# gssales/gaussian-splatting-reflection

Hardware: AMD Instinct MI355X
Metric: train_step_views_per_s (fwd+bwd, 1e6 Gaussians @1080p, surfel rasterizer + reflection path) (higher is better)
Workload: dtype f32

## Files before the change

gaussian-splatting-reflection_amd/csrc/gsr_common.hip:

```cpp
#include "gsr_internal.hpp"
#include <cstdarg>
#include <string>
#include <initializer_list>
#include <vector>
#include <mutex>
#include "gsr_sort.hpp"
#include <rocprim/device/device_scan.hpp>
#include <rocprim/iterator/counting_iterator.hpp>
#include <rocprim/iterator/transform_iterator.hpp>

namespace gsr {

static thread_local char g_err[512] = "";
void set_error(const char* fmt, ...) {
	va_list ap;
	va_start(ap, fmt);
	vsnprintf(g_err, sizeof(g_err), fmt, ap);
	va_end(ap);
}


struct ProfRec {
	int stage;
	hipEvent_t e0, e1;
};
static bool g_prof_on = false;
static std::vector<ProfRec*> g_prof_recs;
static std::vector<ProfRec*> g_prof_free;
static std::mutex g_prof_mu;

StageTimer::StageTimer(int stage_, hipStream_t stream_) : stage(stage_), stream(stream_), rec(nullptr) {
	if (!g_prof_on) return;
	std::lock_guard<std::mutex> lk(g_prof_mu);
	ProfRec* r = nullptr;
	if (!g_prof_free.empty()) {
		r = g_prof_free.back();
		g_prof_free.pop_back();
	} else {
		r = new ProfRec();
		if (hipEventCreate(&r->e0) != hipSuccess || hipEventCreate(&r->e1) != hipSuccess) { delete r; return; }
	}
	r->stage = stage;
	(void)hipEventRecord(r->e0, stream);
	rec = r;
}
StageTimer::~StageTimer() {
	if (!rec) return;
	ProfRec* r = (ProfRec*)rec;
	(void)hipEventRecord(r->e1, stream);
	std::lock_guard<std::mutex> lk(g_prof_mu);
	g_prof_recs.push_back(r);
}

static int g_opt_cull = 1;
int option_cull() { return g_opt_cull; }
static int g_opt_dev = 0;
int option_dev() { return g_opt_dev; }
unsigned long long* dev_pair_counter() {
	static std::mutex mu;
	static unsigned long long* words[64];
	int dev = 0;
	if (hipGetDevice(&dev) != hipSuccess || dev < 0 || dev >= 64) return nullptr;
	std::lock_guard<std::mutex> lk(mu);
	if (!words[dev]) {
		if (hipMalloc((void**)&words[dev], sizeof(unsigned long long)) != hipSuccess) { (void)hipGetLastError(); words[dev] = nullptr; return nullptr; }
		if (hipMemset(words[dev], 0, sizeof(unsigned long long)) != hipSuccess) return nullptr;
	}
	return words[dev];
}
static int g_opt_emit_items = 0;
static int g_opt_mailbox = 1;
static int option_mailbox() { return g_opt_mailbox; }
static int g_opt_sort_driver = GSR_ONESWEEP_DRIVER;
int option_sort_driver() { return GSR_ONESWEEP_DRIVER && g_opt_sort_driver; }

uint32_t higher_msb(uint32_t n) {
	uint32_t msb = sizeof(n) * 4;
	uint32_t step = msb;
	while (step > 1) {
		step /= 2;
		if (n >> msb) msb += step;
		else msb -= step;
	}
	if (n >> msb) msb++;
	return msb;
}

using SortConfig = rocprim::radix_sort_config<rocprim::default_config, rocprim::default_config, rocprim::default_config, 65536>;
#ifndef DEPTH_SORT_BS
#define DEPTH_SORT_BS 1024
#endif
#ifndef DEPTH_SORT_IPT
#define DEPTH_SORT_IPT 4
#endif
#define DEPTH_SORT_SHAPE DEPTH_SORT_BS, DEPTH_SORT_IPT, 8
#define DEPTH_KEY_BITS 31u
#define DEPTH_KEY_PLACES 4u
#ifndef TILE_SORT_IPT
#define TILE_SORT_IPT 16
#endif
#ifndef TILE_SORT_BITS
#define TILE_SORT_BITS 8
#endif
#ifndef TILE_SORT_BS
#define TILE_SORT_BS 1024
#endif
#define TILE_SORT_SHAPE TILE_SORT_BS, TILE_SORT_IPT, TILE_SORT_BITS
#ifndef TILE_SORT_SMALL_FROM
#define TILE_SORT_SMALL_FROM 9000000
#endif
#define TILE_SORT_SHAPE_SMALL TILE_SORT_BS, (TILE_SORT_IPT / 2), TILE_SORT_BITS
#define TILE_SORT_SHAPE_SMALL7 TILE_SORT_BS, (TILE_SORT_IPT / 2), 7
static bool tile_sort_small(size_t R) { return R >= (size_t)TILE_SORT_SMALL_FROM; }
static bool tile_sort_7bit(size_t R, int end_bit) { return tile_sort_small(R) && end_bit > 7 && end_bit <= 14; }
template <class F>
static auto with_tile_sort(size_t R, int end_bit, F&& f) {
	if (tile_sort_7bit(R, end_bit)) return f(RadixSort<TILE_SORT_SHAPE_SMALL7, SortConfig>{});
	if (tile_sort_small(R)) return f(RadixSort<TILE_SORT_SHAPE_SMALL, SortConfig>{});
	return f(RadixSort<TILE_SORT_SHAPE, SortConfig>{});
}
using DepthSort = RadixSort<DEPTH_SORT_SHAPE, SortConfig>;
// ... 518 lines not shown

extern "C" int gsr_set_option(const char* name, int value) {
	if (!name) { set_error("gsr_set_option: NULL option name"); return GSR_E_INVALID; }
	if (std::string(name) == "cull") { g_opt_cull = value ? 1 : 0; return 0; }
	if (std::string(name) == "dev") { g_opt_dev = value; return 0; }
	if (std::string(name) == "emit_items") { g_opt_emit_items = (value == 1 || value == 2) ? value : 0; return 0; }
	if (std::string(name) == "mailbox") { g_opt_mailbox = value ? 1 : 0; return 0; }
	if (std::string(name) == "sort_driver") { g_opt_sort_driver = value ? 1 : 0; return 0; }
	set_error("gsr_set_option: unknown option '%s'", name);
	return GSR_E_INVALID;
}
extern "C" int gsr_profile_enable(int on) {
	std::lock_guard<std::mutex> lk(g_prof_mu);
	for (ProfRec* r : g_prof_recs) g_prof_free.push_back(r);
	g_prof_recs.clear();
	g_prof_on = on != 0;
	return 0;
}
extern "C" int gsr_profile_collect(float* ms_out, int* launches_out) {
	std::lock_guard<std::mutex> lk(g_prof_mu);
	for (int i = 0; i < GSR_STAGE_COUNT; i++) { if (ms_out) ms_out[i] = 0.f; if (launches_out) launches_out[i] = 0; }
	for (ProfRec* r : g_prof_recs) {
		float ms = 0.f;
		if (hipEventSynchronize(r->e1) == hipSuccess && hipEventElapsedTime(&ms, r->e0, r->e1) == hipSuccess) {
			if (ms_out) ms_out[r->stage] += ms;
			if (launches_out) launches_out[r->stage] += 1;
		}
		g_prof_free.push_back(r);
	}
	g_prof_recs.clear();
	return 0;
}

extern "C" int gsr_mark_visible(int P, const float* means3D, const float* viewmatrix, const float* projmatrix, uint8_t* present,
                                void* stream_) {
	(void)projmatrix;
	hipStream_t stream = (hipStream_t)stream_;
	if (P < 0 || (P > 0 && (!means3D || !viewmatrix || !present))) { set_error("gsr_mark_visible: invalid argument"); return GSR_E_INVALID; }
	if (P == 0) return 0;
	mark_visible_kernel<<<(P + 255) / 256, 256, 0, stream>>>(P, means3D, viewmatrix, present);
	GSR_LAUNCH_CHECK(0, stream);
	return 0;
}

extern "C" int gsr_debug_fetch(int variant, const char* name, int P, int R, int width, int height, const void* geom_buffer,
                               const void* binning_buffer, const void* image_buffer, void* dst, void* stream_) {
	hipStream_t stream = (hipStream_t)stream_;
	if ((variant != 0 && variant != 1) || !name || P < 0 || R < 0 || width <= 0 || height <= 0) {
		set_error("gsr_debug_fetch: invalid argument (variant 0 or 1, a name, P >= 0, R >= 0, width, height)");
		return GSR_E_INVALID;
	}
	{
		static const struct { const char* name; int buf; } arrays[] = {
			{"pairs", -1}, {"depths", 0}, {"means2D", 0}, {"tiles_touched", 0}, {"cull", 0}, {"point_offsets", 0}, {"clamped", 0}, {"rgb", 0}, {"geom4", 0},
			{"transMat", 0}, {"cov3D", 0}, {"point_list", 1}, {"blend_mask", 1}, {"keys", 1}, {"ranges", 2}, {"final_T", 2}, {"n_contrib", 2}};
		int buf = -2;
		for (const auto& a : arrays) if (strcmp(a.name, name) == 0) buf = a.buf;
		if (buf == -2 || (strcmp(name, "transMat") == 0 && variant != 0)) { set_error("gsr_debug_fetch: unknown array '%s'", name); return GSR_E_INVALID; }
		const bool reads = buf == -1 || (buf == 0 && P > 0) || (buf == 1 && (R > 0 || strcmp(name, "blend_mask") == 0)) || buf == 2;
		const void* src = buf == 0 ? geom_buffer : buf == 1 ? binning_buffer : buf == 2 ? image_buffer : dst;
		if (reads && (!dst || !src || (strcmp(name, "keys") == 0 && !geom_buffer))) { set_error("gsr_debug_fetch: '%s' needs its workspace buffer and dst", name); return GSR_E_INVALID; }
	}
	const int tiles_x = (width + 15) / 16, tiles_y = (height + 15) / 16;
	const size_t HW = (size_t)width * height, tiles = (size_t)tiles_x * tiles_y;
	const WorkspaceLayout& layout = variant == 0 ? SURFEL_LAYOUT : GAUSS_LAYOUT;
	const int stride = layout.rec_f4 * 4;
	GeomState g = carve_geom((void*)geom_buffer, P, layout, nullptr);
	ImageState im = carve_image((void*)image_buffer, HW, tiles, layout, nullptr);
	BinningState b = carve_binning((void*)binning_buffer, R, tiles, 0, nullptr);
	auto d2d = [&](const void* src, size_t bytes) -> int {
		if (bytes == 0) return 0;
		GSR_HIP_CHECK(hipMemcpyAsync(dst, src, bytes, hipMemcpyDeviceToDevice, stream));
		return 0;
	};
	auto gather = [&](int first, int nf) -> int {
		if (P == 0) return 0;
		gather_rec_kernel<<<(P * nf + 255) / 256, 256, 0, stream>>>(P, (const float*)g.rec, stride, first, nf, (float*)dst);
		GSR_LAUNCH_CHECK(0, stream);
		return 0;
	};
	std::string n(name);
	if (n == "pairs") {
		const unsigned long long* word = dev_pair_counter();
		if (!word) { set_error("gsr_debug_fetch: no pair counter"); return GSR_E_HIP; }
		return d2d(word, sizeof(unsigned long long));
	}
	if (n == "depths") return d2d(g.depths, (size_t)P * 4);
	if (n == "means2D") return gather(0, 2);

	if (n == "tiles_touched") return d2d(g.tiles_touched, (size_t)P * 4);
	if (n == "cull") return d2d(g.bbox, (size_t)P * 32);
	if (n == "point_offsets") {
		if (P == 0) return 0;
		size_t tmp = (size_t)(static_cast<char*>(g.depth_sort_temp) - static_cast<char*>(g.scan_temp));
		GSR_HIP_CHECK(rocprim::inclusive_scan(g.scan_temp, tmp, g.tiles_touched, g.point_offsets, (size_t)P, rocprim::plus<uint32_t>(), stream, false));
		return d2d(g.point_offsets, (size_t)P * 4);
	}
	if (n == "clamped") {
		if (P == 0) return 0;
		widen_clamped_kernel<<<(P + 255) / 256, 256, 0, stream>>>(P, g.clamped, (uint8_t*)dst);
		GSR_LAUNCH_CHECK(0, stream);
		return 0;
	}
	auto pick = [&](std::initializer_list<int> pos) -> int {
		if (P == 0) return 0;
		RecPick pk;
		pk.n = (int)pos.size();
		int i = 0;
		for (int v : pos) pk.pos[i++] = v;
		pick_rec_kernel<<<(P * pk.n + 255) / 256, 256, 0, stream>>>(P, (const float*)g.rec, stride, pk, (float*)dst);
		GSR_LAUNCH_CHECK(0, stream);
		return 0;
	};
	if (n == "rgb") return variant == 0 ? gather(16, 3) : gather(6, 3);
	if (n == "geom4") {
		return variant == 0 ? pick({12, 13, 14, 11}) : gather(2, 4);
	}
	if (n == "transMat" && variant == 0) return pick({2, 4, 6, 3, 5, 7, 8, 9, 10});
	if (n == "cov3D" && variant == 1) { set_error("gsr_debug_fetch: the 3D covariance is not kept by the forward (round 4: the backward recomputes it)"); return GSR_E_INVALID; }
	if (n == "point_list") return d2d(b.point_list, (size_t)R * 4);
	if (n == "blend_mask") return d2d(b.blend_mask, 16 * b.mask_stride * sizeof(unsigned long long));
	if (n == "keys") {
		if (R == 0) return 0;
		rebuild_keys_kernel<<<(R + 255) / 256, 256, 0, stream>>>(R, b.tile_keys, b.point_list, g.depths, (uint64_t*)dst);
		GSR_LAUNCH_CHECK(0, stream);
		return 0;
	}
	if (n == "ranges") return d2d(im.ranges, tiles * 8);
	if (n == "final_T") return d2d(im.final_T, HW * 4 * layout.planes_T);
	if (n == "n_contrib") return d2d(im.n_contrib, HW * 4 * layout.planes_n);
	set_error("gsr_debug_fetch: unknown array '%s'", name);
	return GSR_E_INVALID;
}
```

gaussian-splatting-reflection_amd/csrc/gsr_internal.hpp:

```cpp
#pragma once
#include <cstring>
#include <cstdint>
#include <cstdio>
#include <hip/hip_runtime.h>
#include "../../include/gsr_hip.h"

#define GSR_TILE 16
#define GSR_TILE_PIX 256

namespace gsr {

void set_error(const char* fmt, ...);
#define GSR_HIP_CHECK(expr)                                                                       \
	do {                                                                                          \
		hipError_t _e = (expr);                                                                   \
		if (_e != hipSuccess) {                                                                   \
			gsr::set_error("%s failed: %s (%s:%d)", #expr, hipGetErrorString(_e), __FILE__, __LINE__); \
			return GSR_E_HIP;                                                                     \
		}                                                                                         \
	} while (0)
#define GSR_LAUNCH_CHECK(debug, stream)                                  \
	do {                                                                 \
		GSR_HIP_CHECK(hipGetLastError());                                \
		if (debug) GSR_HIP_CHECK(hipStreamSynchronize(stream));          \
// ... 83 lines not shown
ImageState carve_image(void* buf, size_t HW, size_t tiles, const WorkspaceLayout& layout, size_t* total);
BinningState carve_binning(void* buf, size_t R, size_t tiles, size_t sort_temp_bytes, size_t* total, bool blend_masks = true);
int forward_workspace(gsr_alloc_fn alloc, void* alloc_user, const WorkspaceLayout& layout, size_t P, size_t HW, size_t tiles, GeomState* geom,
                      ImageState* img);

static inline int check_sh_input(const char* entry, int D, int M, const float* shs) {
	if (D < 0 || D > 3 || (shs && (D + 1) * (D + 1) > M)) { set_error("%s: SH degree %d not supported with M=%d", entry, D, M); return GSR_E_INVALID; }
	if (shs && ((M * 3) & 3) == 0 && misaligned16(shs)) {
		set_error("%s: shs (rows of a multiple of 16 bytes) must be 16-byte aligned (float4 accesses); got %p", entry, (const void*)shs);
		return GSR_E_INVALID;
	}
	return 0;
}

struct RasterCam {
	const float* view;
	const float* proj;
	const float* campos;
	int W, H;
	float tan_fovx, tan_fovy, focal_x, focal_y;
};
static inline RasterCam make_cam(const float* view, const float* proj, const float* campos, int W, int H, float tan_fovx, float tan_fovy) {
	RasterCam c;
	c.view = view; c.proj = proj; c.campos = campos; c.W = W; c.H = H;
	c.tan_fovx = tan_fovx; c.tan_fovy = tan_fovy;
	c.focal_y = H / (2.0f * tan_fovy);
	c.focal_x = W / (2.0f * tan_fovx);
	return c;
}

struct BackwardWorkspace { GeomState geom; ImageState img; BinningState bin; int tiles_x, ntiles; };
static inline int backward_prologue(const char* entry, const char* func, const WorkspaceLayout& layout, int P, int M, int R, int width, int height,
                                    bool missing_pointer, const float* shs, const float* dL_dsh, const float* dL_drot, const float* also_aligned,
                                    const char* also_what, void* geom_buffer, void* binning_buffer, void* image_buffer, hipStream_t stream,
                                    BackwardWorkspace* w) {
	if (P < 0 || R < 0 || width <= 0 || height <= 0) { set_error("%s: invalid size", entry); return GSR_E_INVALID; }
	if (P == 0) return 0;
	if (missing_pointer) { set_error("%s: missing required pointer", entry); return GSR_E_INVALID; }
	if (shs && ((M * 3) & 3) == 0) GSR_REQUIRE_ALIGNED16_IN(func, dL_dsh, "dL_dsh");
	GSR_REQUIRE_ALIGNED16_IN(func, dL_drot, "dL_drot");
	GSR_REQUIRE_ALIGNED16_IN(func, also_aligned, also_what);
	w->tiles_x = (width + 15) / 16;
	w->ntiles = w->tiles_x * ((height + 15) / 16);
	w->geom = carve_geom(geom_buffer, P, layout, nullptr);
	w->img = carve_image(image_buffer, (size_t)width * height, w->ntiles, layout, nullptr);
	w->bin = carve_binning(binning_buffer, R, w->ntiles, 0, nullptr);
	GSR_HIP_CHECK(hipMemsetAsync(w->geom.acc, 0, (size_t)P * layout.acc_floats * sizeof(float), stream));
	return 1;
}

int option_cull();
int option_dev();
unsigned long long* dev_pair_counter();
size_t sort_temp_bytes(size_t R, int end_bit);
int run_tile_order(const ImageState& img, size_t tiles, hipStream_t stream);
uint32_t higher_msb(uint32_t n);

int run_binning(gsr_alloc_fn alloc, void* alloc_user, int P, int tiles_x, int tiles_y, const GeomState& geom,
                const ImageState& img, BinningState* out_binning, int prefiltered, int debug, hipStream_t stream, bool blend_masks = true);

int side_gate_wait(hipStream_t stream);
int refl_scratch_check(const char* entry, uint32_t L, int width, int height, const float* scratch, size_t scratch_floats);
int refl_sort_keys_early(uint32_t L, int width, int height, float* scratch, size_t scratch_floats, const uint32_t* sort_keys, int async, bool gated,
                         hipStream_t stream);

}

#ifdef __HIPCC__
namespace gsr {

__device__ __forceinline__ int f2i(float v) { return (int)v; }

__device__ __forceinline__ void get_rect(float px, float py, int max_radius, int gx, int gy, uint32_t& x0, uint32_t& y0,
                                         uint32_t& x1, uint32_t& y1) {
	const float r = (float)max_radius;
	x0 = (uint32_t)min(gx, max(0, f2i((px - r) / 16.0f)));
	y0 = (uint32_t)min(gy, max(0, f2i((py - r) / 16.0f)));
	x1 = (uint32_t)min(gx, max(0, f2i((px + r + 15.0f) / 16.0f)));
	y1 = (uint32_t)min(gy, max(0, f2i((py + r + 15.0f) / 16.0f)));
}

#define GSR_Q1(CTRL, i) "v_add_f32_dpp %" #i ", %" #i ", %" #i " " CTRL " row_mask:0xf bank_mask:0xf\n\t"
#define GSR_DPPB(CTRL, BANK, dst, src) "v_add_f32_dpp %" #dst ", %" #src ", %" #src " " CTRL " row_mask:0xf bank_mask:" BANK "\n\t"
#define GSR_L1(CTRL, d, a, b) GSR_DPPB(CTRL, "0x3", d, a) GSR_DPPB(CTRL, "0xc", d, b)
__device__ __forceinline__ void row_reduce20(const float* v, float* z) {
	float p0, q0, p1, q1, p2, q2, p3, q3, p4, q4;
	asm volatile("s_nop 1\n\t" GSR_L1("row_mirror", 0, 6, 7) GSR_L1("row_mirror", 1, 8, 9) GSR_L1("row_mirror", 2, 10, 11)
	             GSR_L1("row_mirror", 3, 12, 13) GSR_L1("row_mirror", 4, 14, 15) GSR_L1("row_mirror", 5, 16, 17)
	             : "=&v"(p0), "=&v"(q0), "=&v"(p1), "=&v"(q1), "=&v"(p2), "=&v"(q2)
	             : "v"(v[0]), "v"(v[1]), "v"(v[2]), "v"(v[3]), "v"(v[4]), "v"(v[5]), "v"(v[6]), "v"(v[7]), "v"(v[8]), "v"(v[9]), "v"(v[10]), "v"(v[11]));
	asm volatile("s_nop 1\n\t" GSR_L1("row_mirror", 0, 4, 5) GSR_L1("row_mirror", 1, 6, 7) GSR_L1("row_mirror", 2, 8, 9) GSR_L1("row_mirror", 3, 10, 11)
	             : "=&v"(p3), "=&v"(q3), "=&v"(p4), "=&v"(q4)
	             : "v"(v[12]), "v"(v[13]), "v"(v[14]), "v"(v[15]), "v"(v[16]), "v"(v[17]), "v"(v[18]), "v"(v[19]));
#define GSR_L2(d, a, b) GSR_DPPB("row_half_mirror", "0x5", d, a) GSR_DPPB("row_half_mirror", "0xa", d, b)
#define GSR_QA(CTRL) GSR_Q1(CTRL, 0) GSR_Q1(CTRL, 1) GSR_Q1(CTRL, 2) GSR_Q1(CTRL, 3) GSR_Q1(CTRL, 4)
	asm volatile("s_nop 1\n\t" GSR_L2(0, 5, 6) GSR_L2(1, 7, 8) GSR_L2(2, 9, 10) GSR_L2(3, 11, 12) GSR_L2(4, 13, 14)
	             GSR_QA("quad_perm:[2,3,0,1]") GSR_QA("quad_perm:[1,0,3,2]")
	             : "=&v"(z[0]), "=&v"(z[1]), "=&v"(z[2]), "=&v"(z[3]), "=&v"(z[4])
	             : "v"(p0), "v"(q0), "v"(p1), "v"(q1), "v"(p2), "v"(q2), "v"(p3), "v"(q3), "v"(p4), "v"(q4));
}
__device__ __forceinline__ void row_reduce16(const float* v, float* z) {
	float p0, q0, p1, q1, p2, q2, p3, q3;
	asm volatile("s_nop 1\n\t" GSR_L1("row_mirror", 0, 8, 9) GSR_L1("row_mirror", 1, 10, 11) GSR_L1("row_mirror", 2, 12, 13) GSR_L1("row_mirror", 3, 14, 15)
	             GSR_L1("row_mirror", 4, 16, 17) GSR_L1("row_mirror", 5, 18, 19) GSR_L1("row_mirror", 6, 20, 21) GSR_L1("row_mirror", 7, 22, 23)
	             : "=&v"(p0), "=&v"(q0), "=&v"(p1), "=&v"(q1), "=&v"(p2), "=&v"(q2), "=&v"(p3), "=&v"(q3)
	             : "v"(v[0]), "v"(v[1]), "v"(v[2]), "v"(v[3]), "v"(v[4]), "v"(v[5]), "v"(v[6]), "v"(v[7]), "v"(v[8]), "v"(v[9]), "v"(v[10]), "v"(v[11]),
// ... 17 lines not shown
	for (int k = 0; k < N; k++) lds[k * 65 + lane] = v[k];
	wave_lds_sync();
#pragma unroll
	for (int j = 0; j < N; j++) {
		const int e = lane + 64 * j, r = e / N, k = e - r * N;
		if (r < nrows) {
			const float x = lds[k * 65 + r];
			if (ACC) {
				if (x != 0.f) out[e] += x;
			} else {
				out[e] = x;
			}
		}
	}
	wave_lds_sync();
}
template <int N, bool ACC>
__device__ __forceinline__ void wave_store_rows4(float4* lds, const float4* v, float4* __restrict__ out, int pitch, int col0, int nrows, int lane) {
#pragma unroll
	for (int k = 0; k < N; k++) lds[k * 65 + lane] = v[k];
	wave_lds_sync();
#pragma unroll
	for (int j = 0; j < N; j++) {
		const int e = lane + 64 * j, r = e / N, k = e - r * N;
		if (r < nrows) {
			const float4 x = lds[k * 65 + r];
			float4* o = out + (size_t)r * pitch + col0 + k;
			if (ACC) {
				if (x.x != 0.f || x.y != 0.f || x.z != 0.f || x.w != 0.f) {
					const float4 y = *o;
					*o = make_float4(y.x + x.x, y.y + x.y, y.z + x.z, y.w + x.w);
				}
			} else {
				*o = x;
			}
		}
	}
	wave_lds_sync();
}
template <bool ACC> __device__ __forceinline__ void put(float* p, float v) {
	if (ACC) { if (v != 0.f) *p += v; }
	else *p = v;
}
template <bool ACC> __device__ __forceinline__ void put4(float4* p, float a, float b, float c, float d) {
	if (ACC) {
		if (a != 0.f || b != 0.f || c != 0.f || d != 0.f) {
			const float4 r = *p;
			*p = make_float4(r.x + a, r.y + b, r.z + c, r.w + d);
		}
	} else {
		*p = make_float4(a, b, c, d);
	}
}
__device__ __forceinline__ uint32_t ffbl_raw(uint32_t x) {
	uint32_t r;
	asm("v_ffbl_b32 %0, %1" : "=v"(r) : "v"(x));
	return r;
}
__device__ __forceinline__ int row_reduce_slot(int lane) {
	const int q = (lane >> 2) & 3;
	return ((q & 1) << 1) | (q >> 1);
}

typedef unsigned long long lmask;
#define LMASK(cond) __builtin_amdgcn_ballot_w64(cond)
__device__ __forceinline__ float selm(lmask m, float a, float b) {
	float r;
	asm("v_cndmask_b32 %0, %1, %2, %3" : "=v"(r) : "v"(b), "v"(a), "s"(m));
	return r;
}
__device__ __forceinline__ float selm0(lmask m, float a) {
	float r;
	asm("v_cndmask_b32 %0, 0, %1, %2" : "=v"(r) : "v"(a), "s"(m));
	return r;
}
__device__ __forceinline__ uint32_t selmu(lmask m, uint32_t a, uint32_t b) {
	uint32_t r;
	asm("v_cndmask_b32 %0, %1, %2, %3" : "=v"(r) : "v"(b), "v"(a), "s"(m));
	return r;
}

__device__ __forceinline__ float min_raw(float a, float b) {
	float r;
	asm("v_min_f32 %0, %1, %2" : "=v"(r) : "v"(a), "v"(b));
	return r;
}

__device__ __forceinline__ float row_max4(float a, float b, float c, float d) {
	float p, q, z;
	asm volatile("s_nop 1\n\t"
	             "v_max_f32_dpp %0, %2, %2 row_mirror row_mask:0xf bank_mask:0x3\n\t"
	             "v_max_f32_dpp %0, %3, %3 row_mirror row_mask:0xf bank_mask:0xc\n\t"
	             "v_max_f32_dpp %1, %4, %4 row_mirror row_mask:0xf bank_mask:0x3\n\t"
	             "v_max_f32_dpp %1, %5, %5 row_mirror row_mask:0xf bank_mask:0xc\n\t"
	             : "=&v"(p), "=&v"(q) : "v"(a), "v"(b), "v"(c), "v"(d));
	asm volatile("s_nop 1\n\t"
	             "v_max_f32_dpp %0, %1, %1 row_half_mirror row_mask:0xf bank_mask:0x5\n\t"
	             "v_max_f32_dpp %0, %2, %2 row_half_mirror row_mask:0xf bank_mask:0xa\n\t"
	             "s_nop 1\n\t"
	             "v_max_f32_dpp %0, %0, %0 quad_perm:[2,3,0,1] row_mask:0xf bank_mask:0xf\n\t"
	             "s_nop 1\n\t"
	             "v_max_f32_dpp %0, %0, %0 quad_perm:[1,0,3,2] row_mask:0xf bank_mask:0xf\n\t"
	             : "=&v"(z) : "v"(p), "v"(q));
	return z;
}

// ... 63 lines not shown
```

gaussian-splatting-reflection_amd/csrc/gsr_surfel.hip:

```cpp
#include <type_traits>
#include "gsr_internal.hpp"
#include "gsr_tile_walk.hpp"
#include "gsr_sort.hpp"
#include "gsr_math.hpp"
#include "gsr_refl.hpp"

namespace gsr {

#define SA_COLOR 0
#define SA_REFL 3
#define SA_NORMAL 4
#define SA_OPAC 7
#define SA_T 8
#define SA_MEAN2D 17

#define S_NEAR 0.2f
#define S_FAR 100.0f
#define S_FILTER_INV_SQ 2.0f

__device__ __forceinline__ M3 quat_to_rotmat(const float* __restrict__ q, float& w, float& x, float& y, float& z) {
#pragma clang fp contract(off)
	const float s = 1.0f / sqrtf(q[3] * q[3] + q[0] * q[0] + q[1] * q[1] + q[2] * q[2]);
	w = q[0] * s; x = q[1] * s; y = q[2] * s; z = q[3] * s;
	return m3_make(1.f - 2.f * (y * y + z * z), 2.f * (x * y + w * z), 2.f * (x * z - w * y), 2.f * (x * y - w * z),
// ... 24 lines not shown
	float qw, qx, qy, qz;
	const M3 R = quat_to_rotmat(rot, qw, qx, qy, qz);
	const float s0 = mod * scale[0], s1 = mod * scale[1];
	const float L0[3] = {R.m[0][0] * s0, R.m[0][1] * s0, R.m[0][2] * s0};
	const float L1[3] = {R.m[1][0] * s1, R.m[1][1] * s1, R.m[1][2] * s1};
	const float* pm = cam.proj;
	float AB[4][3];
#pragma unroll
	for (int j = 0; j < 4; j++) {
		AB[j][0] = L0[0] * pm[j] + L0[1] * pm[j + 4] + L0[2] * pm[j + 8];
		AB[j][1] = L1[0] * pm[j] + L1[1] * pm[j + 4] + L1[2] * pm[j + 8];
		AB[j][2] = px * pm[j] + py * pm[j + 4] + pz * pm[j + 8] + pm[j + 12];
	}
	const float Wh = (float)(float(cam.W) / 2.0), Wm = (float)(float(cam.W - 1) / 2.0);
	const float Hh = (float)(float(cam.H) / 2.0), Hm = (float)(float(cam.H - 1) / 2.0);
#pragma unroll
	for (int i = 0; i < 3; i++) {
		T.m[0][i] = AB[0][i] * Wh + AB[3][i] * Wm;
		T.m[1][i] = AB[1][i] * Hh + AB[3][i] * Hm;
		T.m[2][i] = AB[3][i];
	}
	const float* vm = cam.view;
	const float nx = R.m[2][0], ny = R.m[2][1], nz = R.m[2][2];
	normal = f3(vm[0] * nx + vm[4] * ny + vm[8] * nz, vm[1] * nx + vm[5] * ny + vm[9] * nz, vm[2] * nx + vm[6] * ny + vm[10] * nz);
}

__device__ __forceinline__ void surfel_cull_record(const M3& T, float cx, float cy, float opa, float4& c0, float4& c1) {
	c0 = make_float4(cx, cy, 0.f, 0.f);
	c1 = make_float4(0.f, cx, cy, -2.0f);
	if (!(opa >= 1.0f / 255.0f)) return;
	const float c2f = 2.0f * logf(255.0f * opa) * 1.05f + 0.1f;
	c1.w = 0.5f * c2f * 1.02f;
	const double ic2 = 1.0 / (double)c2f;
	const double a00 = T.m[0][0], a01 = T.m[0][1], a02 = T.m[0][2];
	const double a10 = T.m[1][0], a11 = T.m[1][1], a12 = T.m[1][2];
	const double a20 = T.m[2][0], a21 = T.m[2][1], a22 = T.m[2][2];
	const double sigma = a20 * a20 + a21 * a21 - a22 * a22 * ic2;
	if (!(sigma < -1e-6 * a22 * a22 * ic2)) return;
	const double sx = a00 * a20 + a01 * a21 - a02 * a22 * ic2, sy = a10 * a20 + a11 * a21 - a12 * a22 * ic2;
	const double Sxx = a00 * a00 + a01 * a01 - a02 * a02 * ic2, Sxy = a00 * a10 + a01 * a11 - a02 * a12 * ic2,
	             Syy = a10 * a10 + a11 * a11 - a12 * a12 * ic2;
	const double is = 1.0 / sigma;
	const double ex = sx * is, ey = sy * is;
	const double g = -is * 1.0404;
	const double Vxx = (Sxx - sx * sx * is) * g + 0.25, Vxy = (Sxy - sx * sy * is) * g, Vyy = (Syy - sy * sy * is) * g + 0.25;
	const double det = Vxx * Vyy - Vxy * Vxy;
	if (!(Vxx > 0.25) || !(Vyy > 0.25) || !(det > 0.0)) return;
	const float fa = (float)(Vyy / det), fb = (float)(-Vxy / det), fc = (float)(Vxx / det);
	if (!(fa > 0.f) || !(fc > 0.f) || !(fa * fc - fb * fb > 0.f) || !(fabsf((float)ex) < 1e7f) || !(fabsf((float)ey) < 1e7f)) return;
	c0 = make_float4((float)ex, (float)ey, fa, fb);
	c1.x = fc;
}

template <bool TRAIN>
__device__ __forceinline__ bool
surfel_preprocess_one(int idx, int D, int M, const float* __restrict__ means, const float* __restrict__ scales, float scale_modifier,
                      const float* __restrict__ rotations, const float* __restrict__ opacities, const float* __restrict__ shs,
                      const float* __restrict__ transMat_precomp, const float* __restrict__ colors_precomp, const float* __restrict__ refl,
                      const uint8_t* __restrict__ env_scope_mask, const RasterCam& cam, int* __restrict__ radii, const GeomState& g, int gx, int gy,
                      int prefiltered, float* __restrict__ gaussian_weights, float4* o) {
#pragma clang fp contract(off)
	radii[idx] = 0;
	if constexpr (TRAIN) gaussian_weights[idx] = 0.f;
	g.tiles_touched[idx] = 0;
	reinterpret_cast<uint2*>(g.rect)[idx] = make_uint2(0u, 0u);
	g.depths[idx] = __int_as_float(0x7f7fffff);
	const float mx = means[3 * idx], my = means[3 * idx + 1], mz = means[3 * idx + 2];
	const float* vm = cam.view;
	const float pvx = vm[0] * mx + vm[4] * my + vm[8] * mz + vm[12];
	const float pvy = vm[1] * mx + vm[5] * my + vm[9] * mz + vm[13];
	const float pvz = vm[2] * mx + vm[6] * my + vm[10] * mz + vm[14];
	if (pvz <= 0.2f) {
		if (prefiltered) g.flags[0] = 1;
		return false;
	}
	M3 T;
	F3 normal;
	if (transMat_precomp == nullptr) {
		compute_transmat(mx, my, mz, scales + 2 * idx, scale_modifier, rotations + 4 * idx, cam, T, normal);
	} else {
#pragma unroll
		for (int c = 0; c < 3; c++)
#pragma unroll
			for (int r = 0; r < 3; r++) T.m[c][r] = transMat_precomp[9 * idx + 3 * c + r];
		normal = f3(0.0f, 0.0f, 1.0f);
	}
	const float cosv = -((pvx * normal.x) + (pvy * normal.y) + (pvz * normal.z));
	if (cosv == 0) return false;
	const float multiplier = cosv > 0 ? 1.f : -1.f;
	normal = f3(multiplier * normal.x, multiplier * normal.y, multiplier * normal.z);
	const float cutoff = 3.0f;
	const float t0 = cutoff * cutoff, t1 = cutoff * cutoff, t2 = -1.0f;
	const float d = t0 * (T.m[2][0] * T.m[2][0]) + t1 * (T.m[2][1] * T.m[2][1]) + t2 * (T.m[2][2] * T.m[2][2]);
	if (d == 0.0f) return false;
	const float inv_d = 1 / d;
	const float f0 = inv_d * t0, f1 = inv_d * t1, f2 = inv_d * t2;
	const float pxi = f0 * (T.m[0][0] * T.m[2][0]) + f1 * (T.m[0][1] * T.m[2][1]) + f2 * (T.m[0][2] * T.m[2][2]);
	const float pyi = f0 * (T.m[1][0] * T.m[2][0]) + f1 * (T.m[1][1] * T.m[2][1]) + f2 * (T.m[1][2] * T.m[2][2]);
	const float h0x = pxi * pxi - (f0 * (T.m[0][0] * T.m[0][0]) + f1 * (T.m[0][1] * T.m[0][1]) + f2 * (T.m[0][2] * T.m[0][2]));
	const float h0y = pyi * pyi - (f0 * (T.m[1][0] * T.m[1][0]) + f1 * (T.m[1][1] * T.m[1][1]) + f2 * (T.m[1][2] * T.m[1][2]));
	const float ex = sqrtf(fmaxf(1e-4f, h0x)), ey = sqrtf(fmaxf(1e-4f, h0y));
	const float radius = ceilf(fmaxf(fmaxf(ex, ey), cutoff * (float)0.707106));
	uint32_t x0, y0, x1, y1;
	get_rect(pxi, pyi, f2i(radius), gx, gy, x0, y0, x1, y1);
	if ((x1 - x0) * (y1 - y0) == 0) return false;

	float cr, cg, cb;
	if (colors_precomp == nullptr) {
		const float dx = mx - cam.campos[0], dy = my - cam.campos[1], dz = mz - cam.campos[2];
		const float len = sqrtf(dx * dx + dy * dy + dz * dz);
		ShRow s;
		load_sh(shs, idx, M, (D + 1) * (D + 1), s);
		const F3 c = sh_eval(D, s, dx / len, dy / len, dz / len);
		if constexpr (TRAIN) g.clamped[idx] = (uint8_t)((c.x < 0 ? 1 : 0) | (c.y < 0 ? 2 : 0) | (c.z < 0 ? 4 : 0));
		cr = fmaxf(c.x, 0.0f); cg = fmaxf(c.y, 0.0f); cb = fmaxf(c.z, 0.0f);
	} else {
		cr = colors_precomp[3 * idx]; cg = colors_precomp[3 * idx + 1]; cb = colors_precomp[3 * idx + 2];
	}
	g.depths[idx] = pvz;
	radii[idx] = f2i(radius);
	g.rect[2 * idx] = x0 | (y0 << 16);
	g.rect[2 * idx + 1] = x1 | (y1 << 16);
	const float maskv = (env_scope_mask != nullptr && env_scope_mask[idx]) ? 1.0f : 0.0f;
	surfel_cull_record(T, pxi, pyi, opacities[idx], o[5], o[6]);
	float4* rec = o;
	rec[0] = make_float4(pxi, pyi, T.m[0][0], T.m[1][0]);
	rec[1] = make_float4(T.m[0][1], T.m[1][1], T.m[0][2], T.m[1][2]);
	rec[2] = make_float4(T.m[2][0], T.m[2][1], T.m[2][2], opacities[idx]);
	rec[3] = make_float4(normal.x, normal.y, normal.z, refl[idx]);
	rec[4] = make_float4(cr, cg, cb, maskv);
	g.tiles_touched[idx] = (y1 - y0) * (x1 - x0);
	return true;
}

#define S_OUT_F4 7
struct CubemapInterleave {
	const float* cubemap;
	float4* rgba;
	uint32_t ntex, LL;
};
template <bool TRAIN>
__global__ void __launch_bounds__(256)
surfel_preprocess_kernel(int P, int D, int M, const float* __restrict__ means, const float* __restrict__ scales, float scale_modifier,
                         const float* __restrict__ rotations, const float* __restrict__ opacities, const float* __restrict__ shs,
                         const float* __restrict__ transMat_precomp, const float* __restrict__ colors_precomp,
                         const float* __restrict__ refl, const uint8_t* __restrict__ env_scope_mask, RasterCam cam, int* __restrict__ radii,
                         GeomState g, int gx, int gy, int prefiltered, float* __restrict__ gaussian_weights, CubemapInterleave ci) {
	const int idx = blockIdx.x * 256 + threadIdx.x;
	for (uint32_t t = (uint32_t)idx; t < ci.ntex; t += gridDim.x * 256u) {
		const uint32_t f = t / ci.LL, r = t - f * ci.LL;
		const float* c = ci.cubemap + (size_t)f * 3 * ci.LL + r;
		ci.rgba[t] = make_float4(c[0], c[ci.LL], c[2 * (size_t)ci.LL], 0.f);
	}
	sort_clear_region(g.depth_sort_temp, g.depth_sort_clear, (size_t)idx, (size_t)gridDim.x * 256u);
	sort_clear_region(g.emit_state, g.emit_state_bytes, (size_t)idx, (size_t)gridDim.x * 256u);
	if (idx == 0) { g.flags[1] = 0; g.flags[2] = 0; g.flags[3] = 0; }
	__shared__ float4 s_out[4][S_REC_F4 * 65];
	const int lane = threadIdx.x & 63;
	float4* so = s_out[threadIdx.x >> 6];
	float4 o[S_OUT_F4];
#pragma unroll
	for (int k = 0; k < S_OUT_F4; k++) o[k] = make_float4(0.f, 0.f, 0.f, 0.f);
	bool live = false;
	if (idx < P)
		live = surfel_preprocess_one<TRAIN>(idx, D, M, means, scales, scale_modifier, rotations, opacities, shs, transMat_precomp, colors_precomp, refl,
		                             env_scope_mask, cam, radii, g, gx, gy, prefiltered, gaussian_weights, o);
	if (__ballot(live) == 0ull) return;
	const int g0 = idx - lane;
	const int ng = min(64, P - g0);
	wave_store_rows4<S_REC_F4, false>(so, o, g.rec + (size_t)g0 * S_REC_F4, S_REC_F4, 0, ng, lane);
	wave_store_rows4<2, false>(so, o + S_REC_F4, g.bbox + (size_t)g0 * 2, 2, 0, ng, lane);
}

typedef float v2f __attribute__((ext_vector_type(2)));
__device__ __forceinline__ v2f mk2(float a, float b) { v2f r; r.x = a; r.y = b; return r; }

struct SurfelRec : TileRec<S_REC_F4> {
	__device__ __forceinline__ v2f xy() const { return mk2(f[0].x, f[0].y); }
	__device__ __forceinline__ v2f TuvX() const { return mk2(f[0].z, f[0].w); }
	__device__ __forceinline__ v2f TuvY() const { return mk2(f[1].x, f[1].y); }
	__device__ __forceinline__ v2f TuvZ() const { return mk2(f[1].z, f[1].w); }
	__device__ __forceinline__ v2f Twxy() const { return mk2(f[2].x, f[2].y); }
	__device__ __forceinline__ float Twz() const { return f[2].z; }
	__device__ __forceinline__ float opac() const { return f[2].w; }
	__device__ __forceinline__ v2f nxy() const { return mk2(f[3].x, f[3].y); }
	__device__ __forceinline__ float nz() const { return f[3].z; }
	__device__ __forceinline__ float refl() const { return f[3].w; }
	__device__ __forceinline__ v2f rg() const { return mk2(f[4].x, f[4].y); }
	__device__ __forceinline__ float b() const { return f[4].z; }
	__device__ __forceinline__ float mask() const { return f[4].w; }
};

#ifndef GSR_BWD_WPE
#define GSR_BWD_WPE 4
#endif
#ifndef GSR_BWD_LIST
#define GSR_BWD_LIST 1
#endif
#ifndef GSR_BWD_UNROLL
#define GSR_BWD_UNROLL 1
#endif
#ifdef GSR_FWD_WPE
#define GSR_FWD_ATTR __attribute__((amdgpu_waves_per_eu(GSR_FWD_WPE, GSR_FWD_WPE)))
#else
#define GSR_FWD_ATTR
#endif

struct SurfelFwdPix {
	float T, C2, M2, distortion, median_depth, median_contributor, maskacc;
	v2f Crg, Nxy, NzR, DM;
	uint32_t last_contributor;
};

template <bool TRAIN>
__device__ __forceinline__ lmask surfel_fwd_pair(const SurfelRec& R, const v2f pix, uint32_t contributor, bool med_live, SurfelFwdPix& st,
                                                 lmask& done, float& wq, bool& grazed) {
	float sx, sy, rho3d, depth, alpha, rho2d;
	{
#pragma clang fp contract(off)
		const v2f Tw = R.Twxy();
		const v2f X = pix * Tw.x - R.TuvX();
		const v2f Y = pix * Tw.y - R.TuvY();
		const v2f Z = pix * R.Twz() - R.TuvZ();
		const v2f a = Y * Z.yx;
// ... 761 lines not shown
	}
	return check_sh_input(entry, D, M, shs);
}
#define SURFEL_FWD_MISSING "missing required input pointer"

static int early_key_sort(const gsr_refl_forward* refl, int width, int height, int R, hipStream_t stream) {
	if (!refl || !refl->sort_keys || !refl->scratch) return 0;
	return refl_sort_keys_early(refl->L, width, height, refl->scratch, refl->scratch_floats, refl->sort_keys, refl->async_sort, R > 0, stream);
}

template <bool TRAIN>
static int surfel_forward(gsr_alloc_fn alloc, void* alloc_user, int P, int D, int M, const float* background, int width, int height,
                          const float* means3D, const uint8_t* env_scope_mask, const float* shs, const float* colors_precomp,
                          const float* refl_strengths, const float* opacities, const float* scales, float scale_modifier,
                          const float* rotations, const float* transMat_precomp, const float* viewmatrix, const float* projmatrix,
                          const float* cam_pos, float tan_fovx, float tan_fovy, int prefiltered, float* out_color, float* out_others,
                          float* out_alpha, float* out_normal_view, float* out_refl_strength_map, int* radii, float* gaussian_weights,
                          const gsr_refl_forward* refl, int debug, hipStream_t stream) {
	const size_t HW = (size_t)width * height;
	int R = 0;
	if (P == 0) {
		float* normal = TRAIN ? out_others + 2 * HW : out_normal_view;
		if (!normal) {
			normal = static_cast<float*>(alloc(alloc_user, GSR_BUF_IMAGE, HW * 3 * 4));
			if (!normal) { set_error("workspace allocation failed (%zu bytes)", HW * 3 * 4); return GSR_E_ALLOC; }
		}
		GSR_HIP_CHECK(hipMemsetAsync(out_color, 0, HW * 3 * 4, stream));
		if (TRAIN) {
			GSR_HIP_CHECK(hipMemsetAsync(out_others, 0, HW * 8 * 4, stream));
		} else {
			GSR_HIP_CHECK(hipMemsetAsync(out_alpha, 0, HW * 4, stream));
			GSR_HIP_CHECK(hipMemsetAsync(normal, 0, HW * 3 * 4, stream));
		}
		GSR_HIP_CHECK(hipMemsetAsync(out_refl_strength_map, 0, HW * 4, stream));
		if (refl && gsr_deferred_reflection_forward_keys(normal, out_color, out_refl_strength_map, refl->cam, refl->cubemap, refl->fail_value, refl->L,
		                                                 width, height, refl->out_final, refl->out_refl_color, refl->out_normal_world, refl->cubemap_rgba,
		                                                 refl->sort_keys, stream) < 0)
			return GSR_E_HIP;
	} else {
		const int tiles_x = (width + 15) / 16, tiles_y = (height + 15) / 16;
		const int ntiles = tiles_x * tiles_y;
		GeomState geom; ImageState img;
		if (const int rc = forward_workspace(alloc, alloc_user, TRAIN ? SURFEL_LAYOUT : SURFEL_LAYOUT.inference(), P, HW, ntiles, &geom, &img); rc < 0) return rc;

		if (prefiltered) GSR_HIP_CHECK(hipMemsetAsync(geom.flags, 0, 4 * sizeof(int), stream));
		const RasterCam cam = make_cam(viewmatrix, projmatrix, cam_pos, width, height, tan_fovx, tan_fovy);
		CubemapInterleave ci{nullptr, nullptr, 0u, 1u};
		SurfelReflFwd rf{};
		if (refl) {
			ci = CubemapInterleave{refl->cubemap, reinterpret_cast<float4*>(refl->cubemap_rgba), 6u * refl->L * refl->L, refl->L * refl->L};
			rf = SurfelReflFwd{refl->cam, refl->cubemap, reinterpret_cast<const float4*>(refl->cubemap_rgba), refl->fail_value, (int)refl->L, 6u * refl->L * refl->L,
			                   refl->out_final, refl->out_refl_color, refl->out_normal_world, refl->sort_keys};
		}
	{ StageTimer st_(GSR_STAGE_PREPROCESS, stream); 	surfel_preprocess_kernel<TRAIN><<<(P + 255) / 256, 256, 0, stream>>>(P, D, M, means3D, scales, scale_modifier, rotations, opacities, shs,
		                                                                     transMat_precomp, colors_precomp, refl_strengths, env_scope_mask, cam, radii, geom,
		                                                                     tiles_x, tiles_y, prefiltered, gaussian_weights, ci); }
		GSR_LAUNCH_CHECK(debug, stream);

		BinningState bin;
		R = run_binning(alloc, alloc_user, P, tiles_x, tiles_y, geom, img, &bin, prefiltered, debug, stream, TRAIN);
		if (R < 0) return R;

	{ StageTimer st_(GSR_STAGE_RENDER_FWD, stream);
		const int nunits = (int)xcd_grid((uint32_t)ntiles * 4u);
		const auto args = [&] { if constexpr (TRAIN) return rf; else return SurfelEvalFwd{rf, out_alpha, out_normal_view}; }();
		auto launch = [&](auto render, auto pairs) {
			render<<<nunits, 64, 0, stream>>>(img.ranges, img.tile_order, bin.point_list, width, height, tiles_x, ntiles, geom.rec, geom.bbox, option_cull(),
			                                  background, TRAIN ? img.final_T : nullptr, TRAIN ? img.n_contrib : nullptr, out_color, out_others,
			                                  out_refl_strength_map, gaussian_weights, bin.blend_mask, bin.mask_stride, args, pairs);
		};
		if (option_dev() & 2) {
			unsigned long long* word = dev_pair_counter();
			if (!word) { set_error("gsr_surfel_forward: no pair counter"); return GSR_E_HIP; }
			launch(refl ? surfel_render_fwd_wave_kernel<true, TRAIN, true> : surfel_render_fwd_wave_kernel<false, TRAIN, true>, PairCount<true>{word, option_dev() & 4});
		} else {
			launch(refl ? surfel_render_fwd_wave_kernel<true, TRAIN> : surfel_render_fwd_wave_kernel<false, TRAIN>, PairCount<false>{});
		} }
		GSR_LAUNCH_CHECK(debug, stream);
	}
	if (const int rc = TRAIN ? early_key_sort(refl, width, height, R, stream) : 0; rc < 0) return rc;
	return R;
}

extern "C" int gsr_surfel_forward_refl(gsr_alloc_fn alloc, void* alloc_user, int P, int D, int M, const float* background, int width, int height,
                                  const float* means3D, const uint8_t* env_scope_mask, const float* shs, const float* colors_precomp,
                                  const float* refl_strengths, const float* opacities, const float* scales, float scale_modifier,
                                  const float* rotations, const float* transMat_precomp, const float* viewmatrix, const float* projmatrix,
                                  const float* cam_pos, float tan_fovx, float tan_fovy, int prefiltered, float* out_color, float* out_others,
                                  float* out_refl_strength_map, int* radii, float* gaussian_weights, const gsr_refl_forward* refl, int debug,
                                  void* stream_) {
	if (!alloc || P < 0 || width <= 0 || height <= 0 || !background || !out_color || !out_others || !out_refl_strength_map) {
		set_error("gsr_surfel_forward: invalid argument");
		return GSR_E_INVALID;
	}
	if (P > 0 && (!gaussian_weights || !opacities)) { set_error("gsr_surfel_forward: " SURFEL_FWD_MISSING); return GSR_E_INVALID; }
	if (const int rc = check_refl_descriptor("gsr_surfel_forward_refl", refl, width, height); rc < 0) return rc;
	if (const int rc = check_surfel_inputs("gsr_surfel_forward", SURFEL_FWD_MISSING, P, D, M, means3D, shs, colors_precomp, refl_strengths, scales, rotations,
	                                       transMat_precomp, viewmatrix, projmatrix, cam_pos, radii); rc < 0) return rc;
	return surfel_forward<true>(alloc, alloc_user, P, D, M, background, width, height, means3D, env_scope_mask, shs, colors_precomp, refl_strengths,
	                            opacities, scales, scale_modifier, rotations, transMat_precomp, viewmatrix, projmatrix, cam_pos, tan_fovx, tan_fovy,
	                            prefiltered, out_color, out_others, nullptr, nullptr, out_refl_strength_map, radii, gaussian_weights, refl, debug,
	                            (hipStream_t)stream_);
}

extern "C" int gsr_surfel_forward(gsr_alloc_fn alloc, void* alloc_user, int P, int D, int M, const float* background, int width, int height,
                                  const float* means3D, const uint8_t* env_scope_mask, const float* shs, const float* colors_precomp,
                                  const float* refl_strengths, const float* opacities, const float* scales, float scale_modifier,
                                  const float* rotations, const float* transMat_precomp, const float* viewmatrix, const float* projmatrix,
                                  const float* cam_pos, float tan_fovx, float tan_fovy, int prefiltered, float* out_color, float* out_others,
// ... 97 lines not shown
```

Before: 549.0.

## Persistent software-pipelined surfel preprocess with prefetched inputs and scalarized camera

Turns the surfel preprocess kernel into a persistent grid sized to CU count times waves-per-EU. Each block loops over batches of Gaussians and double-buffers the per-Gaussian inputs, so the SH row for the next batch is loaded while the current batch is computed. It also adds a specialized PLAIN path for degree-3 SH using float4 loads, pins camera matrices to wave-uniform registers, and caps occupancy at one wave per EU by default. The aim is to hide global-load latency in this memory-bound kernel, at the cost of much lower occupancy and heavier register use from the double-buffered SH rows.

Result: faster. 555.8, median of 6 (+1.3%).

```diff
diff --git a/gaussian-splatting-reflection_amd/csrc/gsr_common.hip b/gaussian-splatting-reflection_amd/csrc/gsr_common.hip
--- a/gaussian-splatting-reflection_amd/csrc/gsr_common.hip
+++ b/gaussian-splatting-reflection_amd/csrc/gsr_common.hip
@@ -67,6 +67,15 @@
 		if (hipMemset(words[dev], 0, sizeof(unsigned long long)) != hipSuccess) return nullptr;
 	}
 	return words[dev];
+}
+int cu_count() {
+	static std::mutex mu;
+	static int cus[64];
+	int dev = 0;
+	if (hipGetDevice(&dev) != hipSuccess || dev < 0 || dev >= 64) return 0;
+	std::lock_guard<std::mutex> lk(mu);
+	if (!cus[dev] && hipDeviceGetAttribute(&cus[dev], hipDeviceAttributeMultiprocessorCount, dev) != hipSuccess) { (void)hipGetLastError(); cus[dev] = 0; }
+	return cus[dev];
 }
 static int g_opt_emit_items = 0;
 static int g_opt_mailbox = 1;
@@ -691,7 +700,7 @@
 	}
 	{
 		static const struct { const char* name; int buf; } arrays[] = {
-			{"pairs", -1}, {"depths", 0}, {"means2D", 0}, {"tiles_touched", 0}, {"cull", 0}, {"point_offsets", 0}, {"clamped", 0}, {"rgb", 0}, {"geom4", 0},
+			{"pairs", -1}, {"pergauss_grid", -1}, {"depths", 0}, {"means2D", 0}, {"tiles_touched", 0}, {"cull", 0}, {"point_offsets", 0}, {"clamped", 0}, {"rgb", 0}, {"geom4", 0},
 			{"transMat", 0}, {"cov3D", 0}, {"point_list", 1}, {"blend_mask", 1}, {"keys", 1}, {"ranges", 2}, {"final_T", 2}, {"n_contrib", 2}};
 		int buf = -2;
 		for (const auto& a : arrays) if (strcmp(a.name, name) == 0) buf = a.buf;
@@ -724,6 +733,13 @@
 		if (!word) { set_error("gsr_debug_fetch: no pair counter"); return GSR_E_HIP; }
 		return d2d(word, sizeof(unsigned long long));
 	}
+	if (n == "pergauss_grid") {
+		const int fwd = variant == 0 ? S_PRE_FWD_WGS : 0, bwd = 0;
+		const uint32_t grids[4] = {(uint32_t)pergauss_grid(P, fwd), (uint32_t)pergauss_grid(P, bwd), (uint32_t)(cu_count() * fwd), (uint32_t)(cu_count() * bwd)};
+		GSR_HIP_CHECK(hipMemcpyAsync(dst, grids, sizeof(grids), hipMemcpyHostToDevice, stream));
+		GSR_HIP_CHECK(hipStreamSynchronize(stream));
+		return 0;
+	}
 	if (n == "depths") return d2d(g.depths, (size_t)P * 4);
 	if (n == "means2D") return gather(0, 2);
 
diff --git a/gaussian-splatting-reflection_amd/csrc/gsr_internal.hpp b/gaussian-splatting-reflection_amd/csrc/gsr_internal.hpp
--- a/gaussian-splatting-reflection_amd/csrc/gsr_internal.hpp
+++ b/gaussian-splatting-reflection_amd/csrc/gsr_internal.hpp
@@ -159,6 +159,17 @@
 int option_cull();
 int option_dev();
 unsigned long long* dev_pair_counter();
+#define PG_BLOCK 256
+#ifndef S_PRE_FWD_WGS
+#define S_PRE_FWD_WGS 1
+#endif
+int cu_count();
+static inline int pergauss_grid(int P, int wgs_per_cu) {
+	const long long nb = ((long long)P + PG_BLOCK - 1) / PG_BLOCK, cap = (long long)cu_count() * wgs_per_cu;
+	if (cap <= 0 || cap >= nb) return (int)nb;
+	const long long trips = (nb + cap - 1) / cap;
+	return (int)((nb + trips - 1) / trips);
+}
 size_t sort_temp_bytes(size_t R, int end_bit);
 int run_tile_order(const ImageState& img, size_t tiles, hipStream_t stream);
 uint32_t higher_msb(uint32_t n);
@@ -282,6 +293,45 @@
 		*p = make_float4(a, b, c, d);
 	}
 }
+__device__ __forceinline__ float wave_uniform(float x) { return __int_as_float(__builtin_amdgcn_readfirstlane(__float_as_int(x))); }
+struct CamRegs {
+	float view[16], proj[16], campos[3];
+	__device__ __forceinline__ explicit CamRegs(const RasterCam& c) {
+#pragma unroll
+		for (int i = 0; i < 16; i++) { view[i] = wave_uniform(c.view[i]); proj[i] = wave_uniform(c.proj[i]); }
+#pragma unroll
+		for (int i = 0; i < 3; i++) campos[i] = wave_uniform(c.campos[i]);
+	}
+	__device__ __forceinline__ RasterCam cam(RasterCam c) const { c.view = view; c.proj = proj; c.campos = campos; return c; }
+};
+template <int N> __device__ __forceinline__ void forget(float (&v)[N]) {
+#pragma unroll
+	for (int k = 0; k < N; k++) asm("" : "=v"(v[k]));
+}
+template <class In, class Load, class Late, class Body>
+__device__ __forceinline__ void pergauss_batches(int P, Load load, Late late, Body body) {
+	const int nb = (int)(((unsigned)P + PG_BLOCK - 1u) / PG_BLOCK), step = (int)gridDim.x, tid = (int)threadIdx.x;
+	int b = (int)blockIdx.x;
+	if (b >= nb) return;
+	auto row = [&](int batch) { return min(min(batch, nb - 1) * PG_BLOCK + tid, P - 1); };
+	In in0, in1;
+	load(in0, row(b));
+	late(in0, row(b));
+	auto thread = [&] { int t = tid; asm volatile("" : "+v"(t)); return t; };
+	for (;;) {
+		int n = b + step;
+		load(in1, row(n));
+		body(in0, b * PG_BLOCK + thread(), [&] { late(in1, row(n)); });
+		if (n >= nb) return;
+		b = n;
+		n = b + step;
+		load(in0, row(n));
+		body(in1, b * PG_BLOCK + thread(), [&] { late(in0, row(n)); });
+		if (n >= nb) return;
+		b = n;
+	}
+}
+
 __device__ __forceinline__ uint32_t ffbl_raw(uint32_t x) {
 	uint32_t r;
 	asm("v_ffbl_b32 %0, %1" : "=v"(r) : "v"(x));
diff --git a/gaussian-splatting-reflection_amd/csrc/gsr_surfel.hip b/gaussian-splatting-reflection_amd/csrc/gsr_surfel.hip
--- a/gaussian-splatting-reflection_amd/csrc/gsr_surfel.hip
+++ b/gaussian-splatting-reflection_amd/csrc/gsr_surfel.hip
@@ -100,20 +100,61 @@
 	c1.x = fc;
 }
 
+struct SurfelIn {
+	float mean[3], scale[2], rot[4], opacity, refl;
+	uint32_t mask;
+	ShRow sh;
+};
+template <bool PLAIN>
+__device__ __forceinline__ void surfel_in_load_sh(SurfelIn& in, int row, int D, int M, const float* __restrict__ shs) {
+	if constexpr (PLAIN) {
+		const float4* r4 = reinterpret_cast<const float4*>(shs) + (size_t)row * 12;
+#pragma unroll
+		for (int q = 0; q < 12; q++) {
+			const float4 t = r4[q];
+			in.sh.v[4 * q + 0] = t.x; in.sh.v[4 * q + 1] = t.y; in.sh.v[4 * q + 2] = t.z; in.sh.v[4 * q + 3] = t.w;
+		}
+	} else {
+		forget(in.sh.v);
+		if (shs != nullptr) load_sh(shs, row, M, (D + 1) * (D + 1), in.sh);
+	}
+}
+template <bool PLAIN>
+__device__ __forceinline__ void surfel_in_load(SurfelIn& in, int row, const float* __restrict__ means, const float* __restrict__ scales,
+                                               const float* __restrict__ rotations, const float* __restrict__ opacities,
+                                               const float* __restrict__ refl, const uint8_t* __restrict__ mask_bytes) {
+	in.mean[0] = means[3 * row]; in.mean[1] = means[3 * row + 1]; in.mean[2] = means[3 * row + 2];
+	if (PLAIN || scales != nullptr) {
+		in.scale[0] = scales[2 * row]; in.scale[1] = scales[2 * row + 1];
+#pragma unroll
+		for (int k = 0; k < 4; k++) in.rot[k] = rotations[4 * row + k];
+	}
+	in.opacity = opacities[row];
+	in.refl = refl[row];
+	in.mask = mask_bytes[row];
+}
+__device__ __forceinline__ F3 surfel_sh_colour(const SurfelIn& in, int D, const RasterCam& cam) {
+#pragma clang fp contract(off)
+	const float mx = in.mean[0], my = in.mean[1], mz = in.mean[2];
+	const float dx = mx - cam.campos[0], dy = my - cam.campos[1], dz = mz - cam.campos[2];
+	const float len = sqrtf(dx * dx + dy * dy + dz * dz);
+	F3 c = sh_eval(D, in.sh, dx / len, dy / len, dz / len);
+	asm volatile("" : "+v"(c.x), "+v"(c.y), "+v"(c.z));
+	return c;
+}
+
 template <bool TRAIN>
 __device__ __forceinline__ bool
-surfel_preprocess_one(int idx, int D, int M, const float* __restrict__ means, const float* __restrict__ scales, float scale_modifier,
-                      const float* __restrict__ rotations, const float* __restrict__ opacities, const float* __restrict__ shs,
-                      const float* __restrict__ transMat_precomp, const float* __restrict__ colors_precomp, const float* __restrict__ refl,
-                      const uint8_t* __restrict__ env_scope_mask, const RasterCam& cam, int* __restrict__ radii, const GeomState& g, int gx, int gy,
-                      int prefiltered, float* __restrict__ gaussian_weights, float4* o) {
+surfel_preprocess_one(const SurfelIn& in, const F3 c, int idx, float scale_modifier, const float* __restrict__ transMat_precomp,
+                      const float* __restrict__ colors_precomp, const uint8_t* __restrict__ env_scope_mask, const RasterCam& cam,
+                      int* __restrict__ radii, const GeomState& g, int gx, int gy, int prefiltered, float* __restrict__ gaussian_weights, float4* o) {
 #pragma clang fp contract(off)
 	radii[idx] = 0;
 	if constexpr (TRAIN) gaussian_weights[idx] = 0.f;
 	g.tiles_touched[idx] = 0;
 	reinterpret_cast<uint2*>(g.rect)[idx] = make_uint2(0u, 0u);
 	g.depths[idx] = __int_as_float(0x7f7fffff);
-	const float mx = means[3 * idx], my = means[3 * idx + 1], mz = means[3 * idx + 2];
+	const float mx = in.mean[0], my = in.mean[1], mz = in.mean[2];
 	const float* vm = cam.view;
 	const float pvx = vm[0] * mx + vm[4] * my + vm[8] * mz + vm[12];
 	const float pvy = vm[1] * mx + vm[5] * my + vm[9] * mz + vm[13];
@@ -125,7 +166,7 @@
 	M3 T;
 	F3 normal;
 	if (transMat_precomp == nullptr) {
-		compute_transmat(mx, my, mz, scales + 2 * idx, scale_modifier, rotations + 4 * idx, cam, T, normal);
+		compute_transmat(mx, my, mz, in.scale, scale_modifier, in.rot, cam, T, normal);
 	} else {
 #pragma unroll
 		for (int c = 0; c < 3; c++)
@@ -155,11 +196,6 @@
 
 	float cr, cg, cb;
 	if (colors_precomp == nullptr) {
-		const float dx = mx - cam.campos[0], dy = my - cam.campos[1], dz = mz - cam.campos[2];
-		const float len = sqrtf(dx * dx + dy * dy + dz * dz);
-		ShRow s;
-		load_sh(shs, idx, M, (D + 1) * (D + 1), s);
-		const F3 c = sh_eval(D, s, dx / len, dy / len, dz / len);
 		if constexpr (TRAIN) g.clamped[idx] = (uint8_t)((c.x < 0 ? 1 : 0) | (c.y < 0 ? 2 : 0) | (c.z < 0 ? 4 : 0));
 		cr = fmaxf(c.x, 0.0f); cg = fmaxf(c.y, 0.0f); cb = fmaxf(c.z, 0.0f);
 	} else {
@@ -169,13 +205,13 @@
 	radii[idx] = f2i(radius);
 	g.rect[2 * idx] = x0 | (y0 << 16);
 	g.rect[2 * idx + 1] = x1 | (y1 << 16);
-	const float maskv = (env_scope_mask != nullptr && env_scope_mask[idx]) ? 1.0f : 0.0f;
-	surfel_cull_record(T, pxi, pyi, opacities[idx], o[5], o[6]);
+	const float maskv = (env_scope_mask != nullptr && in.mask) ? 1.0f : 0.0f;
+	surfel_cull_record(T, pxi, pyi, in.opacity, o[5], o[6]);
 	float4* rec = o;
 	rec[0] = make_float4(pxi, pyi, T.m[0][0], T.m[1][0]);
 	rec[1] = make_float4(T.m[0][1], T.m[1][1], T.m[0][2], T.m[1][2]);
-	rec[2] = make_float4(T.m[2][0], T.m[2][1], T.m[2][2], opacities[idx]);
-	rec[3] = make_float4(normal.x, normal.y, normal.z, refl[idx]);
+	rec[2] = make_float4(T.m[2][0], T.m[2][1], T.m[2][2], in.opacity);
+	rec[3] = make_float4(normal.x, normal.y, normal.z, in.refl);
 	rec[4] = make_float4(cr, cg, cb, maskv);
 	g.tiles_touched[idx] = (y1 - y0) * (x1 - x0);
 	return true;
@@ -187,37 +223,50 @@
 	float4* rgba;
 	uint32_t ntex, LL;
 };
-template <bool TRAIN>
-__global__ void __launch_bounds__(256)
+template <bool TRAIN, bool PLAIN>
+__global__ void __launch_bounds__(PG_BLOCK) __attribute__((amdgpu_waves_per_eu(S_PRE_FWD_WGS, S_PRE_FWD_WGS)))
 surfel_preprocess_kernel(int P, int D, int M, const float* __restrict__ means, const float* __restrict__ scales, float scale_modifier,
                          const float* __restrict__ rotations, const float* __restrict__ opacities, const float* __restrict__ shs,
                          const float* __restrict__ transMat_precomp, const float* __restrict__ colors_precomp,
                          const float* __restrict__ refl, const uint8_t* __restrict__ env_scope_mask, RasterCam cam, int* __restrict__ radii,
                          GeomState g, int gx, int gy, int prefiltered, float* __restrict__ gaussian_weights, CubemapInterleave ci) {
-	const int idx = blockIdx.x * 256 + threadIdx.x;
-	for (uint32_t t = (uint32_t)idx; t < ci.ntex; t += gridDim.x * 256u) {
+	const CamRegs cam_regs(cam);
+	cam = cam_regs.cam(cam);
+	const int tid0 = blockIdx.x * PG_BLOCK + threadIdx.x;
+	const uint32_t nthreads = gridDim.x * (uint32_t)PG_BLOCK;
+	for (uint32_t t = (uint32_t)tid0; t < ci.ntex; t += nthreads) {
 		const uint32_t f = t / ci.LL, r = t - f * ci.LL;
 		const float* c = ci.cubemap + (size_t)f * 3 * ci.LL + r;
 		ci.rgba[t] = make_float4(c[0], c[ci.LL], c[2 * (size_t)ci.LL], 0.f);
 	}
-	sort_clear_region(g.depth_sort_temp, g.depth_sort_clear, (size_t)idx, (size_t)gridDim.x * 256u);
-	sort_clear_region(g.emit_state, g.emit_state_bytes, (size_t)idx, (size_t)gridDim.x * 256u);
-	if (idx == 0) { g.flags[1] = 0; g.flags[2] = 0; g.flags[3] = 0; }
+	sort_clear_region(g.depth_sort_temp, g.depth_sort_clear, (size_t)tid0, (size_t)nthreads);
+	sort_clear_region(g.emit_state, g.emit_state_bytes, (size_t)tid0, (size_t)nthreads);
+	if (tid0 == 0) { g.flags[1] = 0; g.flags[2] = 0; g.flags[3] = 0; }
 	__shared__ float4 s_out[4][S_REC_F4 * 65];
-	const int lane = threadIdx.x & 63;
-	float4* so = s_out[threadIdx.x >> 6];
-	float4 o[S_OUT_F4];
-#pragma unroll
-	for (int k = 0; k < S_OUT_F4; k++) o[k] = make_float4(0.f, 0.f, 0.f, 0.f);
-	bool live = false;
-	if (idx < P)
-		live = surfel_preprocess_one<TRAIN>(idx, D, M, means, scales, scale_modifier, rotations, opacities, shs, transMat_precomp, colors_precomp, refl,
-		                             env_scope_mask, cam, radii, g, gx, gy, prefiltered, gaussian_weights, o);
-	if (__ballot(live) == 0ull) return;
-	const int g0 = idx - lane;
-	const int ng = min(64, P - g0);
-	wave_store_rows4<S_REC_F4, false>(so, o, g.rec + (size_t)g0 * S_REC_F4, S_REC_F4, 0, ng, lane);
-	wave_store_rows4<2, false>(so, o + S_REC_F4, g.bbox + (size_t)g0 * 2, 2, 0, ng, lane);
+	const float* sh_in = colors_precomp == nullptr ? shs : nullptr;
+	const uint8_t* mask_bytes = env_scope_mask != nullptr ? env_scope_mask : reinterpret_cast<const uint8_t*>(opacities);
+	pergauss_batches<SurfelIn>(
+		P, [&](SurfelIn& in, int row) { surfel_in_load<PLAIN>(in, row, means, scales, rotations, opacities, refl, mask_bytes); },
+		[&](SurfelIn& in, int row) { surfel_in_load_sh<PLAIN>(in, row, D, M, sh_in); },
+		[&](const SurfelIn& in, int idx, auto mid) {
+			const int lane = idx & 63;
+			float4* so = s_out[(idx >> 6) & 3];
+			F3 c = f3(0.f, 0.f, 0.f);
+			if (PLAIN || sh_in != nullptr) c = surfel_sh_colour(in, D, cam);
+			mid();
+			float4 o[S_OUT_F4];
+#pragma unroll
+			for (int k = 0; k < S_OUT_F4; k++) o[k] = make_float4(0.f, 0.f, 0.f, 0.f);
+			bool live = false;
+			if (idx < P)
+				live = surfel_preprocess_one<TRAIN>(in, c, idx, scale_modifier, PLAIN ? nullptr : transMat_precomp, PLAIN ? nullptr : colors_precomp,
+				                                    env_scope_mask, cam, radii, g, gx, gy, prefiltered, gaussian_weights, o);
+			if (__ballot(live) == 0ull) return;
+			const int g0 = idx - lane;
+			const int ng = min(64, P - g0);
+			wave_store_rows4<S_REC_F4, false>(so, o, g.rec + (size_t)g0 * S_REC_F4, S_REC_F4, 0, ng, lane);
+			wave_store_rows4<2, false>(so, o + S_REC_F4, g.bbox + (size_t)g0 * 2, 2, 0, ng, lane);
+		});
 }
 
 typedef float v2f __attribute__((ext_vector_type(2)));
@@ -1085,9 +1134,13 @@
 			rf = SurfelReflFwd{refl->cam, refl->cubemap, reinterpret_cast<const float4*>(refl->cubemap_rgba), refl->fail_value, (int)refl->L, 6u * refl->L * refl->L,
 			                   refl->out_final, refl->out_refl_color, refl->out_normal_world, refl->sort_keys};
 		}
-	{ StageTimer st_(GSR_STAGE_PREPROCESS, stream); 	surfel_preprocess_kernel<TRAIN><<<(P + 255) / 256, 256, 0, stream>>>(P, D, M, means3D, scales, scale_modifier, rotations, opacities, shs,
-		                                                                     transMat_precomp, colors_precomp, refl_strengths, env_scope_mask, cam, radii, geom,
-		                                                                     tiles_x, tiles_y, prefiltered, gaussian_weights, ci); }
+	{ StageTimer st_(GSR_STAGE_PREPROCESS, stream);
+		const bool plain = shs != nullptr && colors_precomp == nullptr && M == 16 && D == 3 && scales != nullptr && rotations != nullptr &&
+		                   transMat_precomp == nullptr;
+		auto kern = plain ? surfel_preprocess_kernel<TRAIN, true> : surfel_preprocess_kernel<TRAIN, false>;
+		kern<<<pergauss_grid(P, S_PRE_FWD_WGS), PG_BLOCK, 0, stream>>>(P, D, M, means3D, scales, scale_modifier, rotations, opacities, shs, transMat_precomp,
+		                                                              colors_precomp, refl_strengths, env_scope_mask, cam, radii, geom, tiles_x, tiles_y,
+		                                                              prefiltered, gaussian_weights, ci); }
 		GSR_LAUNCH_CHECK(debug, stream);
 
 		BinningState bin;
```
